# slimgroup/dfno

Hardware: NVIDIA H100
Metric: 3D Navier-Stokes FNO training step (fwd+loss+bwd+Adam) samples/sec, whole job, device-timed, max over ranks (higher is better)
Workload: dtype bf16; 1 GPU; model=FNO3d+t 128^3x20t width 20 modes (12, 12, 12, 10) blocks 4, global_batch=1, seq_len=41943040, parallelism=y-pencil 1x1 (model parallel: field over y, spectral weights over kz), step=forward + DistributedRelativeLpLoss + backward + Adam

## Files before the change

### dfno_b200/csrc/kernels.h

```cpp
#pragma once
#include <cuda_runtime.h>
#include <stdint.h>

namespace dfno {

struct LiftDims {
  int B, Cin, Tin;
  int C, T;
  int X, Y, Z;
};

struct LiftPad {
  int X, Y, Z, T;
};

const char* lift_fwd(const void* x, int x_is_bf16, const float* W1, const float* b1, const float* W2,
                     const float* b2, void* h, LiftDims d, const LiftPad* pad, int num_sms, cudaStream_t s);
const char* lift_bwd(const void* x, int x_is_bf16, const float* W1, const float* b1, const float* W2,
                     const float* b2, const void* dh, float* gW1, float* gb1, float* gW2, float* gb2, float* dx,
                     LiftDims d, const LiftPad* pad, int num_sms, cudaStream_t s);
const char* permute_u32(const void* src, void* dst, int nd, const int* size, const long long* sstr,
                        const long long* dstr, int num_sms, cudaStream_t s);
const char* gelu_probe(const float* x, float* y, float* dy, long long n, cudaStream_t s);
const char* gelu_probe_h2(const float* x, float* y, float* dy, long long n, cudaStream_t s);
// ... 25 lines not shown

const char* p2p_barrier(uint32_t* const* peer_flags, uint32_t* my_flags, int rank, int world, uint32_t epoch,
                        unsigned long long timeout_ns, cudaStream_t s);
const char* p2p_allreduce_small(float* const* peer_bufs, float* out, long long n, int rank, int world,
                                cudaStream_t s);
const char* p2p_sum_f64(double* const* peer_bufs, double* out, int world, cudaStream_t s);

const char* p2p_alltoall(const void* send, const long long* send_off, void* const* peer_recv, const long long* dst_off,
                         int world, int ctas_per_peer, cudaStream_t s);

const char* kreduce_gemm(const void* A, long long lda, int Ma, const void* Bm, long long ldb, int Nb, long long K,
                         float* D, long long ldd, int num_sms, cudaStream_t s);

const char* head_bwd(const void* hcl, long long npos, int C, int CP, const void* W3pad, const void* W3Tpad,
                     const float* b3, const float* W4, const float* dout, int nrl, const int* R, const long long* SR,
                     void* gcl, float* gW3, float* gb3, float* gW4, float* gb4, int num_sms, cudaStream_t stream);

const char* fft_radix(const void* x, void* y, int bf16, int N, long long lines, int inverse, int in_real, int out_real,
                      int one_sided, int m, int num_sms, cudaStream_t s);

const char* spectral_in(const void* h, const void* op1, int n1_pad, int k1_pad, const void* op2, int n2_pad, int k2_pad,
                        const long long* dst_ptrs, int P, long long dst_off, const long long* dstr, int BC, int X,
                        int Yl, int T, int Z, int KZ, int mt, int num_sms, cudaStream_t stream);
const char* spectral_in_check(int n1_pad, int k1_pad, int n2_pad, int k2_pad, int P, long long dst_off, const long long* dstr,
                              int BC, int X, int Yl, int T, int Z, int KZ, int mt, int* cfg );

const char* sq_partials(const float* yh, const float* y, float* part, long long n_per_b, int B, int num_sms, cudaStream_t s);
const char* scaled_diff(const float* yh, const float* y, const float* scale, float* grad, long long n_per_b, int B,
                        int scale_per_b, int num_sms, cudaStream_t s);

const char* spectral_out(const void* U, const void* h, const void* Bop, int n_pad, int k_pad, const float* W,
                         int transpose_w, void* pre, void* out, int B, int C, long long L, int Z, int K1, int gelu,
                         int save_pre, int num_sms, cudaStream_t stream);
const char* dpre_dw(const void* g, void* pre_dpre, const void* h, float* dW, int B, int C, long long L, int Z,
                    int num_sms, cudaStream_t stream);
const char* head_fwd(const void* h, const void* W3aug, const float* w4b4, float* out, int B, int C, long long S,
                     int nrl, const int* R, const long long* SR, const int* lim, int num_sms, cudaStream_t stream);
const char* head_bwd2(const void* h, const void* W3aug, const void* W3T16, const float* W4, const float* dout,
                      long long n_dout, unsigned* amax_ws, void* g, float* gW3, float* gb3, float* gW4, float* gb4,
                      int B, int C, long long S, int nrl, const int* R, const long long* SR, const int* lim,
                      int num_sms, cudaStream_t stream);
const char* head_fwd_multi(const void* h, const void* W3aug, const float* w4b4, float* out, int B, int C, long long S,
                           int O, long long plane, int nrl, const int* R, const long long* SR, const int* lim,
                           int num_sms, cudaStream_t stream);
const char* head_bwd_multi(const void* h, const void* W3aug, const void* W3T16, const float* W4, const float* dout,
                           long long n_dout, unsigned* amax_ws, void* g, float* gW3, float* gb3, float* gW4, float* gb4,
                           int B, int C, long long S, int O, long long plane, int nrl, const int* R,
                           const long long* SR, const int* lim, int num_sms, cudaStream_t stream);

}
```

### dfno_b200/csrc/ops_bindings.cpp

```cpp
#include <torch/extension.h>
#include <ATen/cuda/CUDAContext.h>
#include <c10/cuda/CUDAGuard.h>

#include "kernels.h"

namespace {

int sm_count() {
  static int n = 0;
  if (!n) n = at::cuda::getCurrentDeviceProperties()->multiProcessorCount;
  return n;
}
cudaStream_t cur_stream() { return at::cuda::getCurrentCUDAStream().stream(); }
void check(const char* err, const char* what) { TORCH_CHECK(err == nullptr, what, ": ", err ? err : ""); }
const float* fptr(const at::Tensor& t) {
  TORCH_CHECK(t.is_cuda() && t.scalar_type() == at::kFloat && t.is_contiguous(), "expected contiguous CUDA fp32 tensor");
  return t.data_ptr<float>();
}
float* fptr_mut(at::Tensor& t) { return const_cast<float*>(fptr(t)); }
void* bptr(const at::Tensor& t) {
  TORCH_CHECK(t.is_cuda() && t.scalar_type() == at::kBFloat16, "expected CUDA bf16 tensor");
  return t.data_ptr();
}

// ... 211 lines not shown
  c10::cuda::CUDAGuard guard(x.device());
  at::Tensor y = at::empty_like(x), dy = at::empty_like(x);
  check(dfno::gelu_probe_h2(fptr(x), y.data_ptr<float>(), dy.data_ptr<float>(), x.numel(), cur_stream()), "gelu_probe_h2");
  return {y, dy};
}

void head_bwd(const at::Tensor& hcl, int64_t npos, int64_t C, int64_t CP, const at::Tensor& W3pad,
              const at::Tensor& W3Tpad, const at::Tensor& b3, const at::Tensor& W4, const at::Tensor& dout,
              const std::vector<int64_t>& radices, const std::vector<int64_t>& strides, at::Tensor& gcl,
              at::Tensor& gW3, at::Tensor& gb3, at::Tensor& gW4, at::Tensor& gb4) {
  TORCH_CHECK(radices.size() == strides.size() && !radices.empty() && radices.size() <= 4, "1..4 row digits");
  TORCH_CHECK(W3pad.dim() == 2 && W3pad.size(0) == 128 && W3pad.size(1) == 64 && W3pad.is_contiguous(), "W3pad [128,64]");
  TORCH_CHECK(W3Tpad.dim() == 2 && W3Tpad.size(0) == 32 && W3Tpad.size(1) == 128 && W3Tpad.is_contiguous(), "W3Tpad [32,128]");
  c10::cuda::CUDAGuard guard(hcl.device());
  int R[4]; long long SR[4];
  for (size_t i = 0; i < 4; ++i) { R[i] = i < radices.size() ? static_cast<int>(radices[i]) : 1; SR[i] = i < strides.size() ? strides[i] : 0; }
  check(dfno::head_bwd(bptr(hcl), npos, static_cast<int>(C), static_cast<int>(CP), bptr(W3pad), bptr(W3Tpad), fptr(b3),
                       fptr(W4), fptr(dout), static_cast<int>(radices.size()), R, SR, bptr(gcl), fptr_mut(gW3),
                       fptr_mut(gb3), fptr_mut(gW4), fptr_mut(gb4), sm_count(), cur_stream()), "head_bwd");
}

void fft_radix(const at::Tensor& x, at::Tensor& y, int64_t N, int64_t lines, bool inverse, bool in_real, bool out_real,
               bool one_sided, int64_t m) {
  TORCH_CHECK(x.is_cuda() && y.is_cuda() && x.is_contiguous() && y.is_contiguous(), "contiguous CUDA tensors");
  TORCH_CHECK(x.scalar_type() == y.scalar_type() && (x.scalar_type() == at::kFloat || x.scalar_type() == at::kBFloat16),
              "fp32 or bf16 (same type in and out)");
  c10::cuda::CUDAGuard guard(x.device());
  check(dfno::fft_radix(x.data_ptr(), y.data_ptr(), x.scalar_type() == at::kBFloat16, static_cast<int>(N), lines,
                        inverse, in_real, out_real, one_sided, static_cast<int>(m), sm_count(), cur_stream()), "fft_radix");
}

void spectral_out(const at::Tensor& U, const at::Tensor& h, const at::Tensor& Bop, const at::Tensor& W, bool transpose_w,
                  const c10::optional<at::Tensor>& pre, at::Tensor& out, int64_t B, int64_t C, int64_t L, int64_t Z,
                  int64_t K1, bool gelu, bool save_pre) {
  TORCH_CHECK(Bop.dim() == 2 && Bop.is_contiguous(), "operator must be a contiguous [n_pad, k_pad] tensor");
  c10::cuda::CUDAGuard guard(U.device());
  check(dfno::spectral_out(bptr(U), bptr(h), bptr(Bop), static_cast<int>(Bop.size(0)), static_cast<int>(Bop.size(1)),
                           fptr(W), transpose_w ? 1 : 0, pre ? bptr(*pre) : nullptr, bptr(out), static_cast<int>(B),
                           static_cast<int>(C), L, static_cast<int>(Z), static_cast<int>(K1), gelu ? 1 : 0,
                           save_pre ? 1 : 0, sm_count(), cur_stream()), "spectral_out");
}

void spectral_in(const at::Tensor& h, const at::Tensor& op1, const at::Tensor& op2, const std::vector<int64_t>& dst_ptrs,
                 int64_t dst_off, const std::vector<int64_t>& dstr, int64_t BC, int64_t X, int64_t Yl, int64_t T, int64_t Z,
                 int64_t KZ, int64_t mt) {
  TORCH_CHECK(op1.dim() == 2 && op1.is_contiguous() && op2.dim() == 2 && op2.is_contiguous(), "operators: contiguous [n_pad, k_pad]");
  TORCH_CHECK(!dst_ptrs.empty() && dst_ptrs.size() <= 8 && dstr.size() == 4, "1..8 destinations, 4 strides");
  TORCH_CHECK(h.numel() >= BC * X * Yl * T * Z, "activation smaller than its description");
  c10::cuda::CUDAGuard guard(h.device());
  long long ptrs[8], str[4];
  for (size_t i = 0; i < dst_ptrs.size(); ++i) ptrs[i] = dst_ptrs[i];
  for (size_t i = 0; i < 4; ++i) str[i] = dstr[i];
  check(dfno::spectral_in(bptr(h), bptr(op1), static_cast<int>(op1.size(0)), static_cast<int>(op1.size(1)), bptr(op2),
                          static_cast<int>(op2.size(0)), static_cast<int>(op2.size(1)), ptrs, static_cast<int>(dst_ptrs.size()),
                          dst_off, str, static_cast<int>(BC), static_cast<int>(X), static_cast<int>(Yl), static_cast<int>(T),
                          static_cast<int>(Z), static_cast<int>(KZ), static_cast<int>(mt), sm_count(), cur_stream()),
        "spectral_in");
}

std::string spectral_in_check(int64_t n1_pad, int64_t k1_pad, int64_t n2_pad, int64_t k2_pad, int64_t P, int64_t dst_off,
                              const std::vector<int64_t>& dstr, int64_t BC, int64_t X, int64_t Yl, int64_t T, int64_t Z,
                              int64_t KZ, int64_t mt) {
  TORCH_CHECK(dstr.size() == 4, "4 strides");
  long long str[4];
  for (size_t i = 0; i < 4; ++i) str[i] = dstr[i];
  const char* e = dfno::spectral_in_check(static_cast<int>(n1_pad), static_cast<int>(k1_pad), static_cast<int>(n2_pad),
                                          static_cast<int>(k2_pad), static_cast<int>(P), dst_off, str, static_cast<int>(BC),
                                          static_cast<int>(X), static_cast<int>(Yl), static_cast<int>(T), static_cast<int>(Z),
                                          static_cast<int>(KZ), static_cast<int>(mt), nullptr);
  return e ? std::string(e) : std::string();
}

std::vector<int64_t> spectral_in_config(int64_t n1_pad, int64_t k1_pad, int64_t n2_pad, int64_t k2_pad, int64_t P,
// ... 96 lines not shown
                             cur_stream()), "head_fwd_multi");
}

void head_bwd_multi(const at::Tensor& h, const at::Tensor& W3aug, const at::Tensor& W3T16, const at::Tensor& W4,
                    const at::Tensor& dout, at::Tensor& amax_ws, at::Tensor& g, at::Tensor& gW3, at::Tensor& gb3,
                    at::Tensor& gW4, at::Tensor& gb4, int64_t B, int64_t C, int64_t S, int64_t O, int64_t plane,
                    const std::vector<int64_t>& radices, const std::vector<int64_t>& strides,
                    const std::vector<int64_t>& limits) {
  TORCH_CHECK(W3aug.dim() == 2 && W3aug.size(0) == 128 && W3aug.size(1) == 64 && W3aug.is_contiguous(), "W3aug [128,64]");
  TORCH_CHECK(W3T16.is_cuda() && W3T16.scalar_type() == at::kHalf && W3T16.dim() == 2 && W3T16.size(1) == 128 &&
              W3T16.size(0) == (C + 1 + 15) / 16 * 16 && W3T16.is_contiguous(), "W3T16: fp16 [ceil16(C+1), 128]");
  TORCH_CHECK(W4.numel() == O * 128 && gW4.numel() == O * 128 && gb4.numel() == O, "W4 / dW4 [O, 128], db4 [O]");
  TORCH_CHECK(dout.numel() >= B * O * plane, "dout smaller than B * O * plane");
  TORCH_CHECK(amax_ws.is_cuda() && amax_ws.numel() >= 1 && amax_ws.element_size() == 4, "amax_ws: one 32-bit word");
  c10::cuda::CUDAGuard guard(h.device());
  int R[5], lim[5]; long long SR[5];
  const int* lp = row_digits(radices, strides, limits, R, SR, lim);
  check(dfno::head_bwd_multi(bptr(h), bptr(W3aug), W3T16.data_ptr(), fptr(W4), fptr(dout), dout.numel(),
                             reinterpret_cast<unsigned*>(amax_ws.data_ptr()), bptr(g), fptr_mut(gW3), fptr_mut(gb3),
                             fptr_mut(gW4), fptr_mut(gb4), static_cast<int>(B), static_cast<int>(C), S,
                             static_cast<int>(O), plane, static_cast<int>(radices.size()), R, SR, lp, sm_count(),
                             cur_stream()), "head_bwd_multi");
}

}

void register_ops(pybind11::module& m) {
  m.def("fft_radix", &fft_radix);
  m.def("sq_partials", &sq_partials);
  m.def("scaled_diff", &scaled_diff);
  m.def("spectral_in", &spectral_in);
  m.def("spectral_in_check", &spectral_in_check);
  m.def("spectral_in_config", &spectral_in_config);
  m.def("spectral_out", &spectral_out);
  m.def("dpre_dw", &dpre_dw);
  m.def("head_fwd", &head_fwd, py::arg("h"), py::arg("W3aug"), py::arg("w4b4"), py::arg("out"), py::arg("B"), py::arg("C"),
        py::arg("S"), py::arg("radices"), py::arg("strides"), py::arg("limits") = std::vector<int64_t>{});
  m.def("head_bwd2", &head_bwd2, py::arg("h"), py::arg("W3aug"), py::arg("W3T16"), py::arg("W4"), py::arg("dout"),
        py::arg("amax_ws"), py::arg("g"), py::arg("gW3"), py::arg("gb3"), py::arg("gW4"), py::arg("gb4"), py::arg("B"),
        py::arg("C"), py::arg("S"), py::arg("radices"), py::arg("strides"), py::arg("limits") = std::vector<int64_t>{});
  m.def("head_fwd_multi", &head_fwd_multi, py::arg("h"), py::arg("W3aug"), py::arg("w4b4"), py::arg("out"), py::arg("B"),
        py::arg("C"), py::arg("S"), py::arg("O"), py::arg("plane"), py::arg("radices"), py::arg("strides"),
        py::arg("limits") = std::vector<int64_t>{});
  m.def("head_bwd_multi", &head_bwd_multi, py::arg("h"), py::arg("W3aug"), py::arg("W3T16"), py::arg("W4"),
        py::arg("dout"), py::arg("amax_ws"), py::arg("g"), py::arg("gW3"), py::arg("gb3"), py::arg("gW4"), py::arg("gb4"),
        py::arg("B"), py::arg("C"), py::arg("S"), py::arg("O"), py::arg("plane"), py::arg("radices"), py::arg("strides"),
        py::arg("limits") = std::vector<int64_t>{});
  m.def("lift_fwd", &lift_fwd);
  m.def("lift_bwd", &lift_bwd, py::arg("x"), py::arg("W1"), py::arg("b1"), py::arg("W2"), py::arg("b2"), py::arg("dh"),
        py::arg("gW1"), py::arg("gb1"), py::arg("gW2"), py::arg("gb2"), py::arg("dims"), py::arg("dx") = c10::nullopt);
  m.def("bypass_gelu_fwd", &bypass_gelu_fwd);
  m.def("bypass_gelu_bwd", &bypass_gelu_bwd);
  m.def("bypass_fwd_tc", &bypass_fwd_tc);
  m.def("bypass_bwd_tc", &bypass_bwd_tc);
  m.def("spectral_mix_fwd", &spectral_mix_fwd);
  m.def("spectral_mix_bwd", &spectral_mix_bwd);
  m.def("adam_step", &adam_step, py::arg("p"), py::arg("g"), py::arg("m"), py::arg("v"), py::arg("lr"), py::arg("beta1"),
        py::arg("beta2"), py::arg("eps"), py::arg("weight_decay"), py::arg("step"), py::arg("grad_scale"),
        py::arg("step_dev") = c10::nullopt);
  m.def("adam_step_dev", &adam_step_dev, py::arg("p"), py::arg("g"), py::arg("m"), py::arg("v"), py::arg("hparams"),
        py::arg("step_dev"), py::arg("grad_scale"), py::arg("sumsq") = c10::nullopt, py::arg("norm_out") = c10::nullopt);
  m.def("adam_set_hparams", &adam_set_hparams, py::arg("hparams"), py::arg("lr"), py::arg("beta1"), py::arg("beta2"),
        py::arg("eps"), py::arg("weight_decay"), py::arg("decoupled"), py::arg("max_norm"));
  m.def("sumsq", &sumsq, py::arg("x"), py::arg("out"), py::arg("partials"), py::arg("ticket"));
  m.def("p2p_sum_f64", &p2p_sum_f64);
  m.def("p2p_barrier", &p2p_barrier);
  m.def("p2p_allreduce_small", &p2p_allreduce_small);
// ... 8 lines not shown
```

### dfno_b200/csrc/spectral_out_sm90.cu

```cuda
#include "sm90_ptx.cuh"
#include "kernels.h"
#include "tma_host.h"

namespace dfno {
namespace {

constexpr uint32_t kBlk = 16384;
constexpr int kMaxStagesS = 4;
constexpr int kMaxE = 2;

struct SpecOutParams {
  int B, C, R, RC;
  long long L;
  long long tiles_per_b;
  int Z, nzt;
  int K1, k1blocks, n_pad;
  int transpose_w;
  const float* W;
  int stages, E;
  uint32_t stage_bytes, zbt;
};

template <bool kGelu, bool kPre>
__global__ void __launch_bounds__(128 * kMaxE + 32, 1)
// ... 120 lines not shown
#pragma unroll
          for (int i = 0; i < 8; ++i) {
            const float x0 = __uint_as_float(v[2 * i]), x1 = __uint_as_float(v[2 * i + 1]);
            pk[i] = act ? h2_to_bf16x2(gelu_h2(h2_from_f32(x0, x1))) : pack_bf16x2(x0, x1);
          }
          uint8_t* rowp = myrow + (c0 >> 6) * kBlk;
          const uint32_t j0 = (c0 & 63) >> 3;
          *reinterpret_cast<uint4*>(rowp + ((j0 ^ sw) << 4)) = make_uint4(pk[0], pk[1], pk[2], pk[3]);
          *reinterpret_cast<uint4*>(rowp + (((j0 + 1) ^ sw) << 4)) = make_uint4(pk[4], pk[5], pk[6], pk[7]);
        }
      }
      fence_proxy_async_smem();
      asm volatile("bar.sync %0, 128;" ::"r"(barid) : "memory");
    };
    stage_rows(kGelu && !kPre);
    if (t0) {
      const CUtensorMap* mp = kPre ? &tmP : &tmO;
      for (int zb = 0; zb < zbn; ++zb) tma_store_3d(mp, stg + zb * kBlk, zt * 128 + zb * 64, l0, b * p.C);
      tma_store_commit();
    }
    if (kPre) {
      if (t0) tma_store_wait_read();
      asm volatile("bar.sync %0, 128;" ::"r"(barid) : "memory");
      stage_rows(true);
      if (t0) {
        for (int zb = 0; zb < zbn; ++zb) tma_store_3d(&tmO, stg + zb * kBlk, zt * 128 + zb * 64, l0, b * p.C);
        tma_store_commit();
      }
    }
  }
  if (t0) tma_store_wait_all();
}

}

const char* spectral_out(const void* U, const void* h, const void* Bop, int n_pad, int k_pad, const float* W,
                         int transpose_w, void* pre, void* out, int B, int C, long long L, int Z, int K1, int gelu,
                         int save_pre, int num_sms, cudaStream_t stream) {
  if (C < 1 || C > 64) return "spectral_out: 1 <= C <= 64";
  if (Z % 8 || Z > 256 || K1 % 8) return "spectral_out: need Z % 8 == 0, Z <= 256 and K1 % 8 == 0";
  if (k_pad % 64 || k_pad > 128 || K1 > k_pad || n_pad % 16 || n_pad < Z || n_pad > 256) return "spectral_out: bad operator padding";
  if (L > (1ll << 31) - 256 || static_cast<long long>(B) * C > (1 << 30)) return "spectral_out: tensor too large";
  SpecOutParams p{};
  p.B = B; p.C = C; p.R = 128 / C; p.RC = p.R * C; p.L = L;
  p.tiles_per_b = (L + p.R - 1) / p.R;
  p.Z = Z; p.nzt = (Z + 127) / 128;
  p.K1 = K1; p.k1blocks = k_pad / 64; p.n_pad = n_pad;
  p.transpose_w = transpose_w; p.W = W;
  p.zbt = Z > 64 ? 2 : 1;
  p.stage_bytes = (p.k1blocks + p.zbt) * kBlk;
  const uint32_t fixed = static_cast<uint32_t>(p.k1blocks) * n_pad * 128 + 2 * kBlk + 1024  + 1024 ;
  const uint32_t budget = 227 * 1024;
  auto scratch_bytes = [](int E) { return static_cast<uint32_t>(4 * E * kRowScratchFloats * 4); };
  p.E = kMaxE; p.stages = 0;
  for (int E = kMaxE; E >= 1 && !p.stages; --E)
    for (int st = kMaxStagesS; st >= 2; --st)
      if (st % E == 0 && fixed + st * p.stage_bytes + E * p.zbt * kBlk + scratch_bytes(E) <= budget) {
        p.E = E; p.stages = st; break;
      }
  if (!p.stages) return "spectral_out: tile does not fit shared memory";
  CUtensorMap tmU, tmH, tmB1, tmP, tmO;
  const uint64_t BC = static_cast<uint64_t>(B) * C;
  if (make_map_3d(&tmU, U, K1, L, BC, K1, static_cast<uint64_t>(L) * K1, 64, p.R, C)) return "tensor map (U) failed";
  if (make_map_3d(&tmH, h, Z, L, BC, Z, static_cast<uint64_t>(L) * Z, 64, p.R, C)) return "tensor map (h) failed";
  if (make_map_2d(&tmB1, Bop, k_pad, n_pad, k_pad, 64, n_pad)) return "tensor map (operator) failed";
  if (make_map_3d(&tmP, pre ? pre : out, Z, L, BC, Z, static_cast<uint64_t>(L) * Z, 64, p.R, C)) return "tensor map (pre) failed";
  if (make_map_3d(&tmO, out, Z, L, BC, Z, static_cast<uint64_t>(L) * Z, 64, p.R, C)) return "tensor map (out) failed";
  const uint32_t smem_bytes = fixed + p.stages * p.stage_bytes + p.E * p.zbt * kBlk + scratch_bytes(p.E);
  const long long tiles = p.tiles_per_b * B * p.nzt;
  const int grid = static_cast<int>(tiles < num_sms ? tiles : num_sms);
  const int threads = 128 * p.E + 32;
  const uint32_t dyn = smem_bytes;
  const bool want_pre = gelu && save_pre && pre != nullptr;
#define DFNO_SO_LAUNCH(G, P)                                                                                         \
  do {                                                                                                               \
    static bool attr = false;                                                                                        \
    if (!attr) {                                                                                                     \
      if (cudaFuncSetAttribute(spectral_out_kernel<G, P>, cudaFuncAttributeMaxDynamicSharedMemorySize, 227 * 1024) != \
          cudaSuccess)                                                                                               \
        return "cudaFuncSetAttribute failed";                                                                        \
      attr = true;                                                                                                   \
    }                                                                                                                \
    spectral_out_kernel<G, P><<<grid, threads, dyn, stream>>>(tmU, tmH, tmB1, tmP, tmO, p);                          \
  } while (0)
  if (gelu && want_pre) DFNO_SO_LAUNCH(true, true);
  else if (gelu) DFNO_SO_LAUNCH(true, false);
  else DFNO_SO_LAUNCH(false, false);
#undef DFNO_SO_LAUNCH
  cudaError_t e = cudaGetLastError();
  return e == cudaSuccess ? nullptr : cudaGetErrorString(e);
}

}
```

### dfno_b200/models/fused.py

```python
from __future__ import annotations

import math
import os
from typing import Dict, List, Optional, Sequence, Tuple

import numpy as np
import torch
import torch.distributed as dist
import torch.nn as nn

from ..ops import operators as OPS
from ..ops.gemm import DFT_GEMM_SMEM, ScatterSpec, dft_gemm_fits, dft_gemm_min_smem, pad_operator
from ..parallel.decomposition import balanced_bounds
from ..parallel.partition import Partition

__all__ = ["FusedDistributedFNO", "FusedAdam", "supports", "wants", "EnginePlan", "fold_onto_pencil",
           "SUPPORTED_WIDTHS", "WIDE_WIDTHS"]

SUPPORTED_WIDTHS = (4, 8, 12, 16, 20, 24, 32)
WIDE_WIDTHS = (48, 64)
MAX_OUT = 4
MAX_IN = 16
MAX_N = 256
HBM_BUDGET = 72 * 2 ** 30
# ... 355 lines not shown
                return [(j0, n) + spec.column_part(j0, n) for j0 in range(0, npairs, n)]
            except ValueError:
                continue
        raise ValueError(f"stage {st['name']}: no column split of {npairs} pairs fits {self.max_n}")

    def memory_bytes(self, train: bool = True) -> Dict[str, int]:
        if self.num_blocks is None:
            raise RuntimeError("call finish(num_blocks) first")
        nb, bf, f32 = self.num_blocks, 2, 4
        legacy = not self.fused_pw
        cl = self.npos * self.CP
        out = {
            "parameters": self.n_theta * f32,
            "workspaces": (max(self.n_Z1, self.n_U) + self.n_S1 + self.n_T1 + self.n_S2 + 2 * self.n_S3 + self.n_T2) * bf,
            "staging": (((self.n_S1 + self.n_T1) * bf if self.staged else 0) + self.n_small * f32
                        if self.world > 1 else 0),
            "input_output": self.B * self.Si // self.Ti * self.Cin * self.Tin * f32 + self.O * self.B * self.Si * f32,
        }
        if train and legacy:
            out["saved_activations"] = (2 * nb * self.n_act + nb * self.n_S3 + cl) * bf
            out["backward_workspaces"] = (2 * self.n_act + cl) * bf
        elif train:
            out["saved_activations"] = ((2 * nb + 1) * self.n_act + nb * self.n_S3) * bf
            out["backward_workspaces"] = self.n_act * bf
        if train:
            out["gradients"] = self.n_theta * f32
            out["adam_moments"] = 2 * self.n_theta * f32
        else:
            out["eval_activations"] = ((3 * self.n_act + cl) if legacy else 2 * self.n_act) * bf
        out["total"] = sum(out.values())
        return out

    def cost_model(self, hbm_gbs: float = H100_COPY_GBS, nvlink_gbs: Optional[float] = None,
                   front: bool = False) -> Dict[str, object]:
        if self.num_blocks is None:
            raise RuntimeError("call finish(num_blocks) first")
        nb, bf, f32 = self.num_blocks, 2, 4
        legacy = not self.fused_pw
        P = self.world
        act, cl = self.n_act * bf, self.npos * self.CP * bf
        x_in = self.B * self.Si // self.Ti * self.Cin * self.Tin * f32
        y_out = self.O * self.B * self.Si * f32
        Z1, S1, S2, S3, T2, U = (self.n_Z1 * bf, self.n_S1 * bf, self.n_S2 * bf, self.n_S3 * bf, self.n_T2 * bf,
                                 self.n_U * bf)
        T1 = self.n_T1 // self.mtp * self.mt * bf
        W = self.C * self.C * self.Q * 2 * f32
        off = (P - 1) / P if P > 1 else 0.0
        chain = [("G1a", act + Z1, 0), ("G1b", Z1 + S1, S1 * off), ("G2", S1 + S2, 0), ("G3", S2 + S3, 0),
                 ("iG3", S3 + T2, 0), ("iG2", T2 + T1, T1 * off), ("iG1b", T1 + U, 0)]
        if not self.has_t:
            U = T1
            chain = [("G1a", act + S1, S1 * off)] + chain[2:-1]
        elif front and not legacy:
            chain = [("spectral_in", act + S1, S1 * off)] + chain[2:]
        if not self.has_x:
            chain = [c for c in chain if c[0] not in ("G3", "iG3")]
        if legacy:
            chain.append(("iG1a", U + act, 0))
        if P > 1 and self.staged:
            chain += [("permS1", 2 * S1, 0), ("permT1", 2 * T1, 0)]
        st = [(n, 2 * nb, b, l) for n, b, l in chain]
        st += [("spectral_mix fwd", nb, 2 * S3 + W, 0), ("spectral_mix bwd", nb, 3 * S3 + 2 * W, 0),
               ("lift fwd", 1, act + x_in, 0), ("lift bwd", 1, self.BC * self.Si * bf + x_in, 0),
               ("adam", 1, 7 * self.n_theta * f32, 0)]
        if legacy:
            st += [("iG1a add (bwd)", nb, act, 0), ("bypass fwd", nb, 4 * act, 0), ("bypass bwd", nb, 5 * act, 0),
                   ("head fwd", 1, cl + y_out, 0), ("head bwd", 1, 2 * cl + y_out, 0)]
        else:
            st += [("spectral_out fwd", nb, U + 3 * act, 0), ("spectral_out adj", nb, U + 2 * act, 0),
                   ("dpre_dw", nb, 4 * act, 0),
                   ("head fwd", 1, act + y_out, 0),
                   ("head bwd", 1, 2 * act + 2 * y_out, 0)]
        hbm = sum(c * b for _, c, b, _ in st)
        link = sum(c * l for _, c, _, l in st)
        return {"stages": st, "hbm_bytes": hbm, "nvlink_bytes": link,
                "hbm_floor_ms": hbm / (hbm_gbs * 1e9) * 1e3,
                "nvlink_ms": (link / (nvlink_gbs * 1e9) * 1e3 if link else 0.0) if nvlink_gbs else None}

    def y_map(self) -> List[int]:
        return _storage_map(self.Yg, self.world, self.Yl)

    def kz_map(self) -> List[int]:
        return _storage_map(self.KZg, self.world, self.kzl)

    def operators(self) -> Dict[str, torch.Tensor]:
        X, Y, Z, T = self.X, self.Yg, self.Z, self.T
        f = {
            "G1a": OPS.fwd_real_to_complex(Z, self.mz), "G1b": OPS.fwd_complex(T, self.mt, False),
            "G2": OPS.fwd_complex(Y, self.my), "iG2": OPS.inv_complex(Y, self.my),
            "iG1b": OPS.inv_complex_hermitian(T, self.mt), "iG1a": OPS.inv_complex_to_real(Z, self.mz),
        }
        if self.Y != self.Yg:
            ym = self.y_map()
            f["G2"], f["iG2"] = _pairs_to_storage(f["G2"], ym, 1), _pairs_to_storage(f["iG2"], ym, 0)
        if self.KZ != self.KZg:
            km = self.kz_map()
            f["G1a"], f["iG1a"] = _pairs_to_storage(f["G1a"], km, 0), _pairs_to_storage(f["iG1a"], km, 1)
        mirror = {"G1a": "iG1a", "G1b": "iG1b", "G2": "iG2", "iG2": "G2", "iG1b": "G1b", "iG1a": "G1a"}
        if not self.has_t:
            for k in ("G1b", "iG1b"):
                del f[k], mirror[k]
        if self.has_x:
            f["G3"], f["iG3"] = OPS.fwd_complex(X, self.mx), OPS.inv_complex(X, self.mx)
            mirror.update({"G3": "iG3", "iG3": "G3"})
# ... 133 lines not shown
        self.use_p2p = self.world > 1 if use_p2p is None else (use_p2p and self.world > 1)
        grp = P_x.group
        if self.world > 1:
            self.sym_S1 = SymmetricBuffer(pl.n_S1 * 2, grp, self.rank, self.world, self.device.index)
            self.sym_T1 = SymmetricBuffer(pl.n_T1 * 2, grp, self.rank, self.world, self.device.index)
            self.sym_small = SymmetricBuffer(pl.n_small * 4, grp, self.rank, self.world, self.device.index)
        else:
            self.sym_S1 = self.sym_T1 = self.sym_small = None
        self.barrier = PeerBarrier(grp, self.rank, self.world)

        bf = dict(device=self.device, dtype=torch.bfloat16)
        self.ws = {"Z1U": torch.empty(max(pl.n_Z1, pl.n_U), **bf)} if pl.has_t else {}
        self.ws.update({
            "S1": self.sym_S1.view([pl.n_S1], torch.bfloat16) if self.world > 1 else torch.empty(pl.n_S1, **bf),
            "T1": self.sym_T1.view([pl.n_T1], torch.bfloat16) if self.world > 1 else torch.empty(pl.n_T1, **bf),
            "S2": torch.empty(pl.n_S2, **bf), "S3w": torch.empty(pl.n_S3, **bf),
            "S4": torch.empty(pl.n_S3, **bf), "T2": torch.empty(pl.n_T2, **bf),
        })
        self._saved: Dict[str, torch.Tensor] = {}
        self._train_bufs_ready = False
        self._generation = 0
        st = os.environ.get("DFNO_STAGED_SCATTER")
        if st is not None:
            if st not in ("0", "1"):
                raise ValueError(f"DFNO_STAGED_SCATTER must be 0 or 1, got {st!r}")
            pl.staged = st == "1" and self.world > 1
        self.chain_desc = pl.chain(staged=pl.staged)
        if pl.staged:
            self.ws["S1s"] = self.ws["S1"]
            self.ws["S1"] = torch.empty(pl.n_S1, **bf)
            self.ws["T1s"] = self.ws["T1"]
            self.ws["T1"] = torch.zeros(pl.n_T1, **bf)
        self.front = self._front_plan()

    @property
    def fused_pw(self) -> bool:
        return self.plan.fused_pw

    @property
    def use_tc_bypass(self) -> bool:
        return self.plan.tc_bypass

    def _front_plan(self) -> Optional[dict]:
        pl = self.plan
        if not pl.has_t:
            return None
        P, r = max(self.world, 1), self.rank
        X, Y, Yl, mt, kzl = pl.X, pl.Y, pl.Yl, pl.mt, pl.kzl
        if pl.staged:
            dstr = [Yl * 2, P * X * Yl * 2, mt * P * X * Yl * 2, kzl * mt * P * X * Yl * 2]
            off = r * X * Yl * 2
        else:
            dstr = [Y * 2, X * Y * 2, mt * X * Y * 2, kzl * mt * X * Y * 2]
            off = r * Yl * 2
        if "G1a" not in self.ops or "G1b" not in self.ops:
            return None
        o1, o2 = self.ops["G1a"], self.ops["G1b"]
        why = self._C.spectral_in_check(o1.shape[0], o1.shape[1], o2.shape[0], o2.shape[1], P, off, dstr,
                                        pl.BC, X, Yl, pl.T, pl.Z, pl.KZ, mt)
        if why:
            return None
        return dict(dstr=dstr, off=off, dst="S1s" if pl.staged else "S1")

    def _front(self, src: torch.Tensor, adj: bool) -> None:
        pl, fr = self.plan, self.front
        if self.world > 1:
# ... 100 lines not shown
        else:
            epi = [0, 0, st["ldc"], 0, 0, 0, 0, 0, 0, 0, 0, 0, 1, 1, 0, 0, 0, 0, 1, 0]
            self._C.dft_gemm(A, st["M"], st["K"], st["lda"], self.ops[name], st["N"], epi, [dst.data_ptr()], add,
                             st["ldc"] if add is not None else 0, 0)
        if st.get("barrier_after"):
            self.barrier()

    def _spectral_chain(self, src, dst, block: int, adj: bool, add=None, fuse: Optional[dict] = None,
                        grad: Optional[torch.Tensor] = None) -> None:
        pl = self.plan
        ws = self.ws
        s3 = self._saved["S3"][block] if (self._train_bufs_ready and not self._eval_mode) else ws["S3w"]
        bufs = {"src": src, "Z1": ws.get("Z1U"), "S1": ws["S1"], "S2": ws["S2"],
                "S3": ws["S3w"] if adj else s3, "S4": ws["S4"], "T2": ws["T2"], "T1": ws["T1"],
                "U": ws.get("Z1U"), "dst": dst, "S1s": ws.get("S1s"), "T1s": ws.get("T1s")}
        R = self._seg(f"blocks.{block}.spectral")
        for st in self.chain_desc:
            if self.front is not None and st["name"] in ("G1a", "G1b"):
                if st["name"] == "G1a":
                    self._front(bufs["src"], adj)
                elif st.get("barrier_after"):
                    self.barrier()
            elif st["name"].startswith("perm"):
                self._C.permute_u32(bufs[st["src"]], bufs[st["dst"]], st["size"], st["sstr"], st["dstr"])
            elif st["name"] == "mix":
                if adj:
                    gR = None if grad is None else self._seg(f"blocks.{block}.spectral", grad)
                    self._C.spectral_mix_bwd(s3, R, bufs["S3"], bufs["S4"], gR, getattr(self, "_acc", False), pl.B, pl.C, pl.Q)
                else:
                    self._C.spectral_mix_fwd(bufs["S3"], R, bufs["S4"], pl.B, pl.C, pl.Q)
            elif fuse is not None and st["name"] == "iG1a":
                self._C.spectral_out(bufs[st["src"]], fuse["h"], self.ops[st["op"] + ("_adj" if adj else "")],
                                     fuse["W"], adj, fuse.get("pre"), dst, pl.B, pl.C, pl.X * pl.Yl * pl.T, pl.Z,
                                     st["K"], not adj, fuse.get("pre") is not None)
            else:
                self._gemm(st, bufs, adj, add if st["name"] == "iG1a" else None)

    def _head_operators(self):
        pl = self.plan
        W3 = self._seg("linear3.W")
        w3 = torch.zeros(pl.H, 64, device=self.device, dtype=torch.bfloat16)
        w3[:, :pl.C] = W3.to(torch.bfloat16)
        w3t = torch.zeros(32, pl.H, device=self.device, dtype=torch.bfloat16)
        w3t[:pl.C] = W3.t().to(torch.bfloat16)
        return w3, w3t

    def _head_operators_cm(self):
        pl = self.plan
        W3, b3 = self._seg("linear3.W"), self._seg("linear3.b")
        w3a = torch.zeros(pl.H, 64 if pl.C + 1 <= 64 else 128, device=self.device, dtype=torch.bfloat16)
        w3a[:, :pl.C] = W3.to(torch.bfloat16)
        w3a[:, pl.C] = b3.to(torch.bfloat16)
        w3t = torch.zeros((pl.C + 1 + 15) // 16 * 16, pl.H, device=self.device, dtype=torch.float16)
        w3t[:pl.C] = W3.t().to(torch.bfloat16).to(torch.float16)
        return w3a, w3t

    def _wpad(self, W: torch.Tensor) -> torch.Tensor:
        out = torch.zeros(32, 64, device=self.device, dtype=torch.bfloat16)
        out[:W.shape[0], :W.shape[1]] = W.to(torch.bfloat16)
        return out

    def _w4b4(self) -> torch.Tensor:
        pl = self.plan
        off, _ = pl.segments["linear4.W"]
        assert pl.segments["linear4.b"][0] == off + pl.O * pl.H
        return self.theta.data[off:off + pl.O * (pl.H + 1)]

# ... 95 lines not shown
        if x.dtype not in (torch.float32, torch.bfloat16):
            x = x.float()
        if self.five_d and x.dim() == 5:
            x, dy = x.unsqueeze(2), dy.unsqueeze(2)
        self._eval_mode = False
        hs, pres = self._saved["h"], self._saved["pre"]
        g = self.ws["g"]
        if theta_grad:
            if self.grad_flat is None:
                self.grad_flat = torch.zeros(pl.n_theta, device=self.device, dtype=torch.float32)
            if not (self.accumulate_grads and self.theta.grad is self.grad_flat):
                self.grad_flat[:pl.n_small].zero_()
            self._acc = bool(self.accumulate_grads and self.theta.grad is self.grad_flat)
            gf = gR = self.grad_flat
        else:
            if "g_small" not in self.ws:
                self.ws["g_small"] = torch.empty(pl.n_small, device=self.device, dtype=torch.float32)
            gf, gR = self.ws["g_small"], None
            gf.zero_()
        if pl.fused_pw:
            nb = self.num_blocks
            with _nvtx("dfno.head.bwd"):
                w3a, w3t = self._head_operators_cm()
                R, SR, *lim = self._head_row_digits()
                head_grads = (self._seg("linear3.W", gf), self._seg("linear3.b", gf),
                              self._seg("linear4.W", gf).view(-1), self._seg("linear4.b", gf))
                if pl.O == 1:
                    C_.head_bwd2(hs[nb], w3a, w3t, self._seg("linear4.W").view(-1), dy.contiguous().float(),
                                 self.ws["amax"], g, *head_grads, pl.B, pl.C, pl.S, R, SR, *lim)
                else:
                    C_.head_bwd_multi(hs[nb], w3a, w3t, self._seg("linear4.W").view(-1), dy.contiguous().float(),
                                      self.ws["amax"], g, *head_grads, pl.B, pl.C, pl.S, pl.O, pl.Si, R, SR, *lim)
            L = pl.X * pl.Yl * pl.T
            for k in reversed(range(nb)):
                with _nvtx(f"dfno.block{k}.bwd"):
                    C_.dpre_dw(g, pres[k], hs[k], self._seg(f"blocks.{k}.linear.W", gf), pl.B, pl.C, L, pl.Z)
                    self._spectral_chain(pres[k], g, k, adj=True,
                                         fuse=dict(h=pres[k], W=self._seg(f"blocks.{k}.linear.W")), grad=gR)
        else:
            hcl, dhb, gcl = self._saved["hcl"], self.ws["dhb"], self.ws["gcl"]
            with _nvtx("dfno.head.bwd"):
                self._head_backward(hcl, dy.contiguous().float(), gcl, gf)
            for k in reversed(range(self.num_blocks)):
                last = k == self.num_blocks - 1
                Wb = self._seg(f"blocks.{k}.linear.W")
                gW = self._seg(f"blocks.{k}.linear.W", gf)
                if pl.tc_bypass:
                    C_.bypass_bwd_tc(None if last else g, gcl if last else None, pl.CP, pres[k], hs[k],
                                     self._wpad(Wb.t()), dhb, gW, pl.B, pl.C, pl.S)
                else:
                    C_.bypass_gelu_bwd(None if last else g, gcl if last else None, pl.CP, pres[k], Wb, pres[k], dhb,
                                       pl.B, pl.C, pl.S)
                    if theta_grad:
                        for b in range(pl.B):
                            sl = slice(b * pl.C * pl.S, (b + 1) * pl.C * pl.S)
                            C_.kreduce_gemm(pres[k][sl], pl.S, pl.C, hs[k][sl], pl.S, pl.C, pl.S, gW)
                with _nvtx(f"dfno.block{k}.spectral.bwd"):
                    self._spectral_chain(pres[k], g, k, adj=True, add=dhb, grad=gR)
        dx = torch.empty(x.shape, device=self.device, dtype=torch.float32) if input_grad else None
        C_.lift_bwd(x, self._seg("linear1.W"), self._seg("linear1.b"), self._seg("linear2.W"),
                    self._seg("linear2.b"), g, self._seg("linear1.W", gf), self._seg("linear1.b", gf),
                    self._seg("linear2.W", gf), self._seg("linear2.b", gf), self._lift_dims(), dx)
        self._sync_small_grads(gf[:pl.n_small])
        if theta_grad:
            self.theta.grad = self.grad_flat
        return dx

    def _sync_small_grads(self, small: torch.Tensor) -> None:
        if self.world <= 1:
            return
        if self.use_p2p:
# ... 280 lines not shown
```

Baseline: 17.20 samples/s.

## Fold next block's GELU-grad and bypass dW into adjoint spectral_out kernel

Adds a warp-specialized adjoint spectral_out kernel that also applies the previous block's GELU derivative to produce its dpre, and accumulates the bypass weight gradient via an extra wgmma with h. In the backward loop this replaces the separate dpre_dw pass for all interior blocks, so those activations are not reread from HBM. The cost is a more complex kernel with two consumer warpgroups alternating tiles, extra smem stages and shared-memory atomics for dW. It is only enabled when the shape checks pass.

```diff
diff --git a/dfno_b200/csrc/kernels.h b/dfno_b200/csrc/kernels.h
--- a/dfno_b200/csrc/kernels.h
+++ b/dfno_b200/csrc/kernels.h
@@ -81,6 +81,10 @@
 const char* spectral_out(const void* U, const void* h, const void* Bop, int n_pad, int k_pad, const float* W,
                          int transpose_w, void* pre, void* out, int B, int C, long long L, int Z, int K1, int gelu,
                          int save_pre, int num_sms, cudaStream_t stream);
+const char* spectral_out_adj(const void* U, const void* dpre, const void* Bop, int n_pad, int k_pad, const float* W,
+                             void* pre_prev, void* g, const void* h, float* dW, int B, int C, long long L, int Z, int K1,
+                             int num_sms, cudaStream_t stream);
+const char* spectral_out_adj_check(int n_pad, int k_pad, int C, int Z, int K1, int dpre, int dw);
 const char* dpre_dw(const void* g, void* pre_dpre, const void* h, float* dW, int B, int C, long long L, int Z,
                     int num_sms, cudaStream_t stream);
 const char* head_fwd(const void* h, const void* W3aug, const float* w4b4, float* out, int B, int C, long long S,
diff --git a/dfno_b200/csrc/ops_bindings.cpp b/dfno_b200/csrc/ops_bindings.cpp
--- a/dfno_b200/csrc/ops_bindings.cpp
+++ b/dfno_b200/csrc/ops_bindings.cpp
@@ -267,13 +267,30 @@
 
 void spectral_out(const at::Tensor& U, const at::Tensor& h, const at::Tensor& Bop, const at::Tensor& W, bool transpose_w,
                   const c10::optional<at::Tensor>& pre, at::Tensor& out, int64_t B, int64_t C, int64_t L, int64_t Z,
-                  int64_t K1, bool gelu, bool save_pre) {
+                  int64_t K1, bool gelu, bool save_pre, const c10::optional<at::Tensor>& pre_prev,
+                  const c10::optional<at::Tensor>& h_dw, const c10::optional<at::Tensor>& dW) {
   TORCH_CHECK(Bop.dim() == 2 && Bop.is_contiguous(), "operator must be a contiguous [n_pad, k_pad] tensor");
   c10::cuda::CUDAGuard guard(U.device());
+  if (pre_prev || h_dw || dW) {
+    TORCH_CHECK(transpose_w && !gelu, "pre_prev / h_dw / dW: adjoint only");
+    TORCH_CHECK(!dW || (dW->scalar_type() == at::kFloat && dW->numel() >= C * C), "dW: fp32 [C, C]");
+    check(dfno::spectral_out_adj(bptr(U), bptr(h), bptr(Bop), static_cast<int>(Bop.size(0)),
+                                 static_cast<int>(Bop.size(1)), fptr(W), pre_prev ? bptr(*pre_prev) : nullptr, bptr(out),
+                                 h_dw ? bptr(*h_dw) : nullptr, dW ? const_cast<float*>(fptr(*dW)) : nullptr, static_cast<int>(B),
+                                 static_cast<int>(C), L, static_cast<int>(Z), static_cast<int>(K1), sm_count(),
+                                 cur_stream()), "spectral_out_adj");
+    return;
+  }
   check(dfno::spectral_out(bptr(U), bptr(h), bptr(Bop), static_cast<int>(Bop.size(0)), static_cast<int>(Bop.size(1)),
                            fptr(W), transpose_w ? 1 : 0, pre ? bptr(*pre) : nullptr, bptr(out), static_cast<int>(B),
                            static_cast<int>(C), L, static_cast<int>(Z), static_cast<int>(K1), gelu ? 1 : 0,
                            save_pre ? 1 : 0, sm_count(), cur_stream()), "spectral_out");
+}
+
+std::string spectral_out_adj_check(int64_t n_pad, int64_t k_pad, int64_t C, int64_t Z, int64_t K1, bool dpre, bool dw) {
+  const char* e = dfno::spectral_out_adj_check(static_cast<int>(n_pad), static_cast<int>(k_pad), static_cast<int>(C),
+                                               static_cast<int>(Z), static_cast<int>(K1), dpre ? 1 : 0, dw ? 1 : 0);
+  return e ? std::string(e) : std::string();
 }
 
 void spectral_in(const at::Tensor& h, const at::Tensor& op1, const at::Tensor& op2, const std::vector<int64_t>& dst_ptrs,
@@ -436,7 +453,11 @@
   m.def("spectral_in", &spectral_in);
   m.def("spectral_in_check", &spectral_in_check);
   m.def("spectral_in_config", &spectral_in_config);
-  m.def("spectral_out", &spectral_out);
+  m.def("spectral_out", &spectral_out, py::arg("U"), py::arg("h"), py::arg("Bop"), py::arg("W"), py::arg("transpose_w"),
+        py::arg("pre"), py::arg("out"), py::arg("B"), py::arg("C"), py::arg("L"), py::arg("Z"), py::arg("K1"),
+        py::arg("gelu"), py::arg("save_pre"), py::arg("pre_prev") = c10::nullopt, py::arg("h_dw") = c10::nullopt,
+        py::arg("dW") = c10::nullopt);
+  m.def("spectral_out_adj_check", &spectral_out_adj_check);
   m.def("dpre_dw", &dpre_dw);
   m.def("head_fwd", &head_fwd, py::arg("h"), py::arg("W3aug"), py::arg("w4b4"), py::arg("out"), py::arg("B"), py::arg("C"),
         py::arg("S"), py::arg("radices"), py::arg("strides"), py::arg("limits") = std::vector<int64_t>{});
diff --git a/dfno_b200/csrc/spectral_out_sm90.cu b/dfno_b200/csrc/spectral_out_sm90.cu
--- a/dfno_b200/csrc/spectral_out_sm90.cu
+++ b/dfno_b200/csrc/spectral_out_sm90.cu
@@ -176,6 +176,238 @@
   if (t0) tma_store_wait_all();
 }
 
+constexpr int kAdjE = 2;
+
+template <bool kDpre, bool kDw>
+__global__ void __launch_bounds__(128 * kAdjE + 32, 1)
+spectral_out_adj_kernel(const __grid_constant__ CUtensorMap tmU, const __grid_constant__ CUtensorMap tmD,
+                        const __grid_constant__ CUtensorMap tmB1, const __grid_constant__ CUtensorMap tmO,
+                        const __grid_constant__ CUtensorMap tmHw, const SpecOutParams p, float* dW) {
+  extern __shared__ __align__(1024) uint8_t smem[];
+  uint8_t* s_b1 = smem;
+  uint8_t* s_a2 = s_b1 + static_cast<uint32_t>(p.k1blocks) * p.n_pad * 128;
+  uint8_t* s_ring = s_a2 + 2 * kBlk;
+  uint64_t* bars = reinterpret_cast<uint64_t*>(s_ring + p.stages * p.stage_bytes);
+  uint64_t* full = bars;
+  uint64_t* empty = bars + 4;
+  uint64_t* bfull = bars + 8;
+  const uint32_t o_d = p.k1blocks * kBlk, o_p = o_d + kBlk, o_h = o_p + (kDpre ? kBlk : 0);
+
+  const int warp = __shfl_sync(0xffffffffu, static_cast<int>(threadIdx.x >> 5), 0), lane = threadIdx.x & 31;
+  const long long num_tiles = p.tiles_per_b * p.B * p.nzt;
+
+  {
+    uint4* z0 = reinterpret_cast<uint4*>(s_a2);
+    const uint32_t nz = (2 * kBlk + p.stages * p.stage_bytes) / 16;
+    for (uint32_t i = threadIdx.x; i < nz; i += blockDim.x) z0[i] = make_uint4(0, 0, 0, 0);
+  }
+  if (threadIdx.x == 0) {
+    tma_prefetch_desc(&tmU); tma_prefetch_desc(&tmD); tma_prefetch_desc(&tmB1);
+    tma_prefetch_desc(&tmO); if (kDw) tma_prefetch_desc(&tmHw);
+    for (int s = 0; s < p.stages; ++s) { mbar_init(&full[s], 1); mbar_init(&empty[s], kAdjE); }
+    mbar_init(bfull, 1);
+    fence_barrier_init();
+  }
+  __syncthreads();
+  for (int idx = threadIdx.x; idx < p.C * p.C * p.R; idx += blockDim.x) {
+    const int a = idx / (p.C * p.R);
+    const int rem = idx - a * (p.C * p.R);
+    const int b = rem / p.R, r = rem - b * p.R;
+    const float w = p.W[b * p.C + a];
+    const int m = a * p.R + r, k = b * p.R + r;
+    const uint32_t off = (k >> 6) * kBlk + m * 128 + (((((k & 63) >> 3) ^ (m & 7)) << 4) | ((k & 7) << 1));
+    *reinterpret_cast<__nv_bfloat16*>(s_a2 + off) = __float2bfloat16(w);
+  }
+  fence_proxy_async_smem();
+  __syncthreads();
+
+  if (warp == 4 * kAdjE) {
+    if (lane == 0) {
+      mbar_arrive_expect_tx(bfull, static_cast<uint32_t>(p.k1blocks) * p.n_pad * 128);
+      for (int kb = 0; kb < p.k1blocks; ++kb) tma_load_2d(s_b1 + kb * p.n_pad * 128, &tmB1, bfull, kb * 64, 0);
+      const uint32_t boxes = p.k1blocks + 1 + (kDpre ? 1 : 0) + (kDw ? 1 : 0);
+      uint32_t s = 0, ph = 0;
+      for (long long tile = blockIdx.x; tile < num_tiles; tile += gridDim.x) {
+        const int zb = static_cast<int>(tile % p.nzt);
+        const long long lt = (tile / p.nzt) % p.tiles_per_b;
+        const int b = static_cast<int>(tile / (p.nzt * p.tiles_per_b));
+        const int l0 = static_cast<int>(lt * p.R);
+        mbar_wait(&empty[s], ph ^ 1);
+        mbar_arrive_expect_tx(&full[s], boxes * p.RC * 128);
+        uint8_t* dst = s_ring + s * p.stage_bytes;
+        for (int kb = 0; kb < p.k1blocks; ++kb) tma_load_3d(dst + kb * kBlk, &tmU, &full[s], kb * 64, l0, b * p.C);
+        tma_load_3d(dst + o_d, &tmD, &full[s], zb * 64, l0, b * p.C);
+        if (kDpre) tma_load_3d(dst + o_p, &tmO, &full[s], zb * 64, l0, b * p.C);
+        if (kDw) tma_load_3d(dst + o_h, &tmHw, &full[s], zb * 64, l0, b * p.C);
+        if (++s == static_cast<uint32_t>(p.stages)) { s = 0; ph ^= 1; }
+      }
+    }
+    return;
+  }
+
+  const int q = warp & 3, g = warp >> 2;
+  const bool t0 = q == 0 && lane == 0;
+  const uint32_t barid = 1 + g;
+  const int k1steps = (p.K1 + 15) >> 4;
+  const int k2steps = (p.RC + 15) >> 4;
+  const uint32_t b1_addr = smem_u32(s_b1), a2_addr = smem_u32(s_a2);
+  mbar_wait(bfull, 0);
+  float acc[64];
+  float accw[kDw ? 64 : 1];
+  long long n = 0;
+  for (long long tile = blockIdx.x; tile < num_tiles; tile += gridDim.x, ++n) {
+    const bool own = n % kAdjE == g;
+    const uint32_t s = static_cast<uint32_t>(n % p.stages);
+    const int zb = static_cast<int>(tile % p.nzt);
+    const long long lt = (tile / p.nzt) % p.tiles_per_b;
+    const int b = static_cast<int>(tile / (p.nzt * p.tiles_per_b));
+    const int ncols = min(64, p.Z - zb * 64);
+    const int ntp = (ncols + 15) & ~15;
+    const int l0 = static_cast<int>(lt * p.R);
+    uint8_t* st = s_ring + s * p.stage_bytes;
+    const uint32_t a1 = smem_u32(st);
+    mbar_wait(&full[s], (n / p.stages) & 1);
+    if (!own) {
+      if constexpr (kDw) {
+        wgmma_fence();
+        const int ksteps = ntp >> 4;
+        for (int kk = 0; kk < ksteps; ++kk)
+          wgmma_m64n128k16_bf16<0, 0>(accw, gdesc_k128(a1 + o_d + g * 8192 + kk * 32), gdesc_k128(a1 + o_h + kk * 32),
+                                      (n > 0 || kk > 0) ? 1u : 0u);
+        wgmma_commit();
+      }
+      if constexpr (kDpre) {
+        uint8_t* pt = st + o_p;
+        const int t = threadIdx.x & 127;
+        for (int i0 = t; i0 < p.RC * 8; i0 += 2 * 128) {
+          uint4 P[2];
+#pragma unroll
+          for (int u = 0; u < 2; ++u)
+            if (i0 + u * 128 < p.RC * 8) P[u] = *reinterpret_cast<const uint4*>(pt + (i0 + u * 128) * 16);
+#pragma unroll
+          for (int u = 0; u < 2; ++u)
+            if (i0 + u * 128 < p.RC * 8) {
+              uint4 G;
+              G.x = h2_bits(gelu_vg_h2(bf16x2_to_h2(P[u].x)).grad);
+              G.y = h2_bits(gelu_vg_h2(bf16x2_to_h2(P[u].y)).grad);
+              G.z = h2_bits(gelu_vg_h2(bf16x2_to_h2(P[u].z)).grad);
+              G.w = h2_bits(gelu_vg_h2(bf16x2_to_h2(P[u].w)).grad);
+              *reinterpret_cast<uint4*>(pt + (i0 + u * 128) * 16) = G;
+            }
+        }
+        asm volatile("bar.sync 3, %0;" ::"n"(128 * kAdjE) : "memory");
+      }
+      if constexpr (kDw) {
+        wgmma_wait<0>();
+        acc_fence(accw);
+      }
+      if (t0) mbar_arrive(&empty[s]);
+      continue;
+    }
+    {
+      wgmma_fence();
+      const uint32_t b1 = b1_addr + zb * 64 * 128;
+      for (int ks = 0; ks < k1steps; ++ks) {
+        const uint32_t kb = ks >> 2, kk = ks & 3;
+        wg_mma128<false, 0, 0>(acc, ntp, gdesc_k128(a1 + kb * kBlk + kk * 32), 8192,
+                               gdesc_k128(b1 + kb * (p.n_pad * 128) + kk * 32), ks > 0 ? 1u : 0u);
+      }
+      for (int ks = 0; ks < k2steps; ++ks) {
+        const uint32_t kb = ks >> 2, kk = ks & 3;
+        wg_mma128<false, 0, 1>(acc, ntp, gdesc_k128(a2_addr + kb * kBlk + kk * 32), 8192,
+                               gdesc_mn128(a1 + o_d + ks * 2048, kBlk, 1024), 1u);
+      }
+      if constexpr (kDw) {
+        const int ksteps = ntp >> 4;
+        for (int kk = 0; kk < ksteps; ++kk)
+          wgmma_m64n128k16_bf16<0, 0>(accw, gdesc_k128(a1 + o_d + g * 8192 + kk * 32), gdesc_k128(a1 + o_h + kk * 32),
+                                      (n > 0 || kk > 0) ? 1u : 0u);
+      }
+      wgmma_commit();
+      wgmma_wait<0>();
+      acc_fence(acc);
+      if constexpr (kDw) acc_fence(accw);
+    }
+    if (kDpre)
+      asm volatile("bar.sync 3, %0;" ::"n"(128 * kAdjE) : "memory");
+    else
+      asm volatile("bar.sync %0, 128;" ::"r"(barid) : "memory");
+    {
+      uint8_t* ot = st + (kDpre ? o_p : 0);
+#pragma unroll
+      for (int h = 0; h < 2; ++h)
+#pragma unroll
+        for (int eh = 0; eh < 2; ++eh) {
+          const int m = 64 * h + 16 * q + (lane >> 2) + 8 * eh;
+          uint8_t* row = ot + m * 128 + 4 * (lane & 3);
+          uint32_t gw[8];
+          if (kDpre) {
+#pragma unroll
+            for (int j = 0; j < 8; ++j)
+              gw[j] = 8 * j < ncols ? *reinterpret_cast<const uint32_t*>(row + ((j ^ (m & 7)) << 4)) : 0u;
+          }
+#pragma unroll
+          for (int j = 0; j < 8; ++j) {
+            if (8 * j < ncols) {
+              const float* a = acc + 32 * h + 4 * j + 2 * eh;
+              uint32_t v = pack_bf16x2(a[0], a[1]);
+              if (kDpre) {
+                const float2 gr = __half22float2(h2_of_bits(gw[j]));
+                const float2 gg = unpack_bf16x2(v);
+                v = pack_bf16x2(gg.x * gr.x, gg.y * gr.y);
+              }
+              *reinterpret_cast<uint32_t*>(row + ((j ^ (m & 7)) << 4)) = v;
+            }
+          }
+        }
+    }
+    fence_proxy_async_smem();
+    asm volatile("bar.sync %0, 128;" ::"r"(barid) : "memory");
+    if (t0) {
+      tma_store_3d(&tmO, st + (kDpre ? o_p : 0), zb * 64, l0, b * p.C);
+      tma_store_commit();
+      tma_store_wait_read();
+      mbar_arrive(&empty[s]);
+    }
+  }
+  if (t0) tma_store_wait_all();
+  if constexpr (kDw) {
+    float* s_dw = reinterpret_cast<float*>(s_ring);
+    asm volatile("bar.sync 3, %0;" ::"n"(128 * kAdjE) : "memory");
+    for (int i = threadIdx.x; i < p.C * p.C; i += 128 * kAdjE) s_dw[i] = 0.f;
+    asm volatile("bar.sync 3, %0;" ::"n"(128 * kAdjE) : "memory");
+    if (n > 0) {
+      const int m0 = 64 * g + 16 * q + (lane >> 2), k0 = 2 * (lane & 3);
+#pragma unroll
+      for (int j = 0; j < 16; ++j)
+#pragma unroll
+        for (int e = 0; e < 4; ++e) {
+          const int m = m0 + 8 * (e >> 1), k = 8 * j + k0 + (e & 1);
+          if (m < p.RC && k < p.RC) {
+            const int o = m / p.R, i = k / p.R;
+            if (m - o * p.R == k - i * p.R) atomicAdd(&s_dw[o * p.C + i], accw[4 * j + e]);
+          }
+        }
+    }
+    asm volatile("bar.sync 3, %0;" ::"n"(128 * kAdjE) : "memory");
+    if (num_tiles > blockIdx.x)
+      for (int i = threadIdx.x; i < p.C * p.C; i += 128 * kAdjE) atomicAdd(dW + i, s_dw[i]);
+  }
+}
+
+uint32_t spectral_out_adj_smem(int k1blocks, int n_pad, bool dpre, bool dw, int* stages_out, uint32_t* stage_bytes_out) {
+  const uint32_t stage_bytes = (k1blocks + 1 + (dpre ? 1 : 0) + (dw ? 1 : 0)) * kBlk;
+  const uint32_t fixed = static_cast<uint32_t>(k1blocks) * n_pad * 128 + 2 * kBlk + 1024  + 1024 ;
+  for (int st = kMaxStagesS; st >= 2; --st) {
+    if (fixed + st * stage_bytes <= 227u * 1024) {
+      if (stages_out) *stages_out = st;
+      if (stage_bytes_out) *stage_bytes_out = stage_bytes;
+      return fixed + st * stage_bytes;
+    }
+  }
+  return 0;
+}
+
 }
 
 const char* spectral_out(const void* U, const void* h, const void* Bop, int n_pad, int k_pad, const float* W,
@@ -235,4 +467,61 @@
   return e == cudaSuccess ? nullptr : cudaGetErrorString(e);
 }
 
-}
+const char* spectral_out_adj_check(int n_pad, int k_pad, int C, int Z, int K1, int dpre, int dw) {
+  if (C < 1 || C > 64) return "spectral_out_adj: 1 <= C <= 64";
+  if (Z % 8 || Z > 256 || K1 % 8) return "spectral_out_adj: need Z % 8 == 0, Z <= 256 and K1 % 8 == 0";
+  if (k_pad % 64 || k_pad > 128 || K1 > k_pad || n_pad % 16 || n_pad < Z || n_pad > 256)
+    return "spectral_out_adj: bad operator padding";
+  if (!dpre && !dw) return "spectral_out_adj: nothing to fold (use spectral_out)";
+  if (!spectral_out_adj_smem(k_pad / 64, n_pad, dpre != 0, dw != 0, nullptr, nullptr))
+    return "spectral_out_adj: two ring stages do not fit shared memory";
+  return nullptr;
+}
+
+const char* spectral_out_adj(const void* U, const void* dpre, const void* Bop, int n_pad, int k_pad, const float* W,
+                             void* pre_prev, void* g, const void* h, float* dW, int B, int C, long long L, int Z, int K1,
+                             int num_sms, cudaStream_t stream) {
+  const bool kd = pre_prev != nullptr, kw = dW != nullptr;
+  if (kw != (h != nullptr)) return "spectral_out_adj: h and dW go together";
+  if (const char* e = spectral_out_adj_check(n_pad, k_pad, C, Z, K1, kd, kw)) return e;
+  if (!kd && !g) return "spectral_out_adj: no output";
+  if (L > (1ll << 31) - 256 || static_cast<long long>(B) * C > (1 << 30)) return "spectral_out_adj: tensor too large";
+  SpecOutParams p{};
+  p.B = B; p.C = C; p.R = 128 / C; p.RC = p.R * C; p.L = L;
+  p.tiles_per_b = (L + p.R - 1) / p.R;
+  p.Z = Z; p.nzt = (Z + 63) / 64;
+  p.K1 = K1; p.k1blocks = k_pad / 64; p.n_pad = n_pad;
+  p.transpose_w = 1; p.W = W;
+  p.E = kAdjE;
+  const uint32_t smem_bytes = spectral_out_adj_smem(p.k1blocks, n_pad, kd, kw, &p.stages, &p.stage_bytes);
+  CUtensorMap tmU, tmD, tmB1, tmO, tmHw;
+  const uint64_t BC = static_cast<uint64_t>(B) * C;
+  const uint64_t LZ = static_cast<uint64_t>(L) * Z;
+  if (make_map_3d(&tmU, U, K1, L, BC, K1, static_cast<uint64_t>(L) * K1, 64, p.R, C)) return "tensor map (U) failed";
+  if (make_map_3d(&tmD, dpre, Z, L, BC, Z, LZ, 64, p.R, C)) return "tensor map (dpre) failed";
+  if (make_map_2d(&tmB1, Bop, k_pad, n_pad, k_pad, 64, n_pad)) return "tensor map (operator) failed";
+  if (make_map_3d(&tmO, kd ? pre_prev : g, Z, L, BC, Z, LZ, 64, p.R, C)) return "tensor map (out) failed";
+  if (make_map_3d(&tmHw, kw ? h : dpre, Z, L, BC, Z, LZ, 64, p.R, C)) return "tensor map (h) failed";
+  const long long tiles = p.tiles_per_b * B * p.nzt;
+  const int grid = static_cast<int>(tiles < num_sms ? tiles : num_sms);
+  const int threads = 128 * kAdjE + 32;
+#define DFNO_SOA_LAUNCH(D, WW)                                                                                        \
+  do {                                                                                                               \
+    static bool attr = false;                                                                                        \
+    if (!attr) {                                                                                                     \
+      if (cudaFuncSetAttribute(spectral_out_adj_kernel<D, WW>, cudaFuncAttributeMaxDynamicSharedMemorySize,          \
+                               227 * 1024) != cudaSuccess)                                                           \
+        return "cudaFuncSetAttribute failed";                                                                        \
+      attr = true;                                                                                                   \
+    }                                                                                                                \
+    spectral_out_adj_kernel<D, WW><<<grid, threads, smem_bytes, stream>>>(tmU, tmD, tmB1, tmO, tmHw, p, dW);         \
+  } while (0)
+  if (kd && kw) DFNO_SOA_LAUNCH(true, true);
+  else if (kd) DFNO_SOA_LAUNCH(true, false);
+  else DFNO_SOA_LAUNCH(false, true);
+#undef DFNO_SOA_LAUNCH
+  cudaError_t e = cudaGetLastError();
+  return e == cudaSuccess ? nullptr : cudaGetErrorString(e);
+}
+
+}
diff --git a/dfno_b200/models/fused.py b/dfno_b200/models/fused.py
--- a/dfno_b200/models/fused.py
+++ b/dfno_b200/models/fused.py
@@ -411,7 +411,7 @@
         return out
 
     def cost_model(self, hbm_gbs: float = H100_COPY_GBS, nvlink_gbs: Optional[float] = None,
-                   front: bool = False) -> Dict[str, object]:
+                   front: bool = False, fold_bwd: bool = False) -> Dict[str, object]:
         if self.num_blocks is None:
             raise RuntimeError("call finish(num_blocks) first")
         nb, bf, f32 = self.num_blocks, 2, 4
@@ -446,9 +446,13 @@
             st += [("iG1a add (bwd)", nb, act, 0), ("bypass fwd", nb, 4 * act, 0), ("bypass bwd", nb, 5 * act, 0),
                    ("head fwd", 1, cl + y_out, 0), ("head bwd", 1, 2 * cl + y_out, 0)]
         else:
-            st += [("spectral_out fwd", nb, U + 3 * act, 0), ("spectral_out adj", nb, U + 2 * act, 0),
-                   ("dpre_dw", nb, 4 * act, 0),
-                   ("head fwd", 1, act + y_out, 0),
+            st += [("spectral_out fwd", nb, U + 3 * act, 0)]
+            if fold_bwd and nb > 1:
+                st += [("spectral_out adj+dpre", 1, U + 3 * act, 0), ("spectral_out adj+dpre+dW", nb - 2, U + 4 * act, 0),
+                       ("spectral_out adj+dW", 1, U + 3 * act, 0), ("dpre_dw", 1, 4 * act, 0)]
+            else:
+                st += [("spectral_out adj", nb, U + 2 * act, 0), ("dpre_dw", nb, 4 * act, 0)]
+            st += [("head fwd", 1, act + y_out, 0),
                    ("head bwd", 1, 2 * act + 2 * y_out, 0)]
         hbm = sum(c * b for _, c, b, _ in st)
         link = sum(c * l for _, c, _, l in st)
@@ -648,6 +652,15 @@
             self.ws["T1s"] = self.ws["T1"]
             self.ws["T1"] = torch.zeros(pl.n_T1, **bf)
         self.front = self._front_plan()
+        self.fold_bwd = self._fold_bwd_plan()
+
+    def _fold_bwd_plan(self) -> bool:
+        pl = self.plan
+        if not pl.fused_pw or "iG1a_adj" not in self.ops:
+            return False
+        op = self.ops["iG1a_adj"]
+        K1 = next(st["K"] for st in self.chain_desc if st["name"] == "iG1a")
+        return not self._C.spectral_out_adj_check(op.shape[0], op.shape[1], pl.C, pl.Z, K1, True, True)
 
     @property
     def fused_pw(self) -> bool:
@@ -814,7 +827,8 @@
             elif fuse is not None and st["name"] == "iG1a":
                 self._C.spectral_out(bufs[st["src"]], fuse["h"], self.ops[st["op"] + ("_adj" if adj else "")],
                                      fuse["W"], adj, fuse.get("pre"), dst, pl.B, pl.C, pl.X * pl.Yl * pl.T, pl.Z,
-                                     st["K"], not adj, fuse.get("pre") is not None)
+                                     st["K"], not adj, fuse.get("pre") is not None, fuse.get("pre_prev"),
+                                     fuse.get("h_dw"), fuse.get("dW"))
             else:
                 self._gemm(st, bufs, adj, add if st["name"] == "iG1a" else None)
 
@@ -976,11 +990,17 @@
                     C_.head_bwd_multi(hs[nb], w3a, w3t, self._seg("linear4.W").view(-1), dy.contiguous().float(),
                                       self.ws["amax"], g, *head_grads, pl.B, pl.C, pl.S, pl.O, pl.Si, R, SR, *lim)
             L = pl.X * pl.Yl * pl.T
+            fold = self.fold_bwd and nb > 1
             for k in reversed(range(nb)):
                 with _nvtx(f"dfno.block{k}.bwd"):
-                    C_.dpre_dw(g, pres[k], hs[k], self._seg(f"blocks.{k}.linear.W", gf), pl.B, pl.C, L, pl.Z)
-                    self._spectral_chain(pres[k], g, k, adj=True,
-                                         fuse=dict(h=pres[k], W=self._seg(f"blocks.{k}.linear.W")), grad=gR)
+                    fuse = dict(h=pres[k], W=self._seg(f"blocks.{k}.linear.W"))
+                    if k == nb - 1 or not fold:
+                        C_.dpre_dw(g, pres[k], hs[k], self._seg(f"blocks.{k}.linear.W", gf), pl.B, pl.C, L, pl.Z)
+                    else:
+                        fuse.update(h_dw=hs[k], dW=self._seg(f"blocks.{k}.linear.W", gf))
+                    if fold and k > 0:
+                        fuse["pre_prev"] = pres[k - 1]
+                    self._spectral_chain(pres[k], g, k, adj=True, fuse=fuse, grad=gR)
         else:
             hcl, dhb, gcl = self._saved["hcl"], self.ws["dhb"], self.ws["gcl"]
             with _nvtx("dfno.head.bwd"):
```

New measurement: 17.97 samples/s (median of 6 runs). +4.5%, better.
